# actuday6418/ray-tracer-s8

Hardware: NVIDIA B200
Metric: Mrays/s (higher is better)
Workload: dtype f32

## Files before the change

ray-tracer-s8_b200/csrc/rt_kernels.cu:

```cuda
#include "rt_trace.cuh"
#include "rt_host.h"

#include <algorithm>
#include <cstdio>
#include <cstdlib>
#include <cstring>

namespace rtb {

constexpr int SMEM_TPB = 1024;
constexpr int OUT_SLOTS = 4;
constexpr int TILE_PIX = TILE_W * TILE_H;
constexpr int TILE_BYTES = TILE_PIX * 3;
constexpr uint32_t KEY_FREE = 0xffffffffu;

__device__ __forceinline__ uint32_t smem_u32(const void* p) { return (uint32_t)__cvta_generic_to_shared(p); }
__device__ __forceinline__ void mbar_init(unsigned long long* bar, uint32_t count) {
    asm volatile("mbarrier.init.shared::cta.b64 [%0], %1;" ::"r"(smem_u32(bar)), "r"(count) : "memory");
    asm volatile("fence.mbarrier_init.release.cluster;" ::: "memory");
}
__device__ __forceinline__ void mbar_expect_tx(unsigned long long* bar, uint32_t bytes) {
    asm volatile("mbarrier.arrive.expect_tx.shared::cta.b64 _, [%0], %1;" ::"r"(smem_u32(bar)), "r"(bytes) : "memory");
}
__device__ __forceinline__ void bulk_g2s(void* dst_smem, const void* src_gmem, uint32_t bytes, unsigned long long* bar) {
// ... 20 lines not shown
    unsigned long long* done;
    uint32_t width, out_row0, row0, slab_tile_rows;
};
__device__ __forceinline__ uint32_t slab_of_row(const OutDesc& od, uint32_t y) { return ((y - od.row0) / TILE_H) / od.slab_tile_rows; }

__device__ __forceinline__ void release_count(unsigned long long* done, uint32_t slab, uint32_t cnt) {
    asm volatile("red.release.sys.global.add.u64 [%0], %1;" ::"l"(done + slab), "l"((unsigned long long)cnt) : "memory");
}
__device__ __forceinline__ void count_pixels(const OutDesc& od, uint32_t slab, uint32_t cnt, uint32_t* cntw) {
    if (!od.done || cnt == 0) return;
    if (cntw && (*reinterpret_cast<volatile uint32_t*>(cntw) >> 24) == slab) atomicAdd(cntw, cnt);
    else release_count(od.done, slab, cnt);
}

__device__ __noinline__ void complete_tile(const OutDesc od, const uint8_t* st, uint32_t x0, uint32_t y0, uint32_t valid,
                                           uint32_t hold, uint32_t* cntw) {
    const bool vec = valid == 0xffffffffu && ((od.width & 7u) == 0) && ((reinterpret_cast<uintptr_t>(od.out) & 7u) == 0);
    if (vec) {
#pragma unroll 1
        for (uint32_t r = 0; r < (uint32_t)TILE_H; r++) {
            uint2* dst = reinterpret_cast<uint2*>(od.out + ((size_t)(y0 + r - od.out_row0) * od.width + x0) * 3);
            const uint2* src = reinterpret_cast<const uint2*>(st + r * 24);
            const uint2 v0 = src[0], v1 = src[1], v2 = src[2];
            dst[0] = v0; dst[1] = v1; dst[2] = v2;
        }
    } else {
        for (uint32_t m = valid; m; m &= m - 1u) {
            const uint32_t j = (uint32_t)__ffs(m) - 1u;
            uint8_t* dst = od.out + ((size_t)(y0 + (j >> 3) - od.out_row0) * od.width + x0 + (j & 7u)) * 3;
            dst[0] = st[j * 3 + 0]; dst[1] = st[j * 3 + 1]; dst[2] = st[j * 3 + 2];
        }
    }
    count_pixels(od, slab_of_row(od, y0), (uint32_t)__popc(valid) - hold, cntw);
}

__device__ __noinline__ void evict_tile(const OutDesc od, const uint8_t* st, uint32_t x0, uint32_t y0, uint32_t mask, uint32_t hold,
                                        uint32_t* cntw) {
    const int lane = threadIdx.x & 31;
    if ((mask >> lane) & 1u) {
        const size_t off = ((size_t)(y0 + (lane >> 3) - od.out_row0) * od.width + x0 + (lane & 7)) * 3;
        od.out[off + 0] = st[lane * 3 + 0];
        od.out[off + 1] = st[lane * 3 + 1];
        od.out[off + 2] = st[lane * 3 + 2];
    }
    __syncwarp();
    if (lane == 0) count_pixels(od, slab_of_row(od, y0), (uint32_t)__popc(mask) - hold, cntw);
}

__device__ __noinline__ void store_pixel(const OutDesc od, uint32_t x, uint32_t y, uint32_t rgb, bool count, uint32_t* cntw) {
    const size_t off = ((size_t)(y - od.out_row0) * od.width + x) * 3;
    od.out[off + 0] = (uint8_t)rgb;
    od.out[off + 1] = (uint8_t)(rgb >> 8);
    od.out[off + 2] = (uint8_t)(rgb >> 16);
    if (count) count_pixels(od, slab_of_row(od, y), 1u, cntw);
}

constexpr uint32_t L_HAVE = 1u;           constexpr uint32_t W_TILES_LEFT = 1u;
constexpr uint32_t L_FINISHED = 2u;       constexpr uint32_t W_IN_TAIL = 2u;
                                          constexpr int W_SLOT_SHIFT = 4;
constexpr uint32_t L_REDO = 8u;           constexpr int W_NEXT_SHIFT = 8;
constexpr int L_SLOT_SHIFT = 4;
constexpr uint32_t L_SECOND = 128u;

template <int ISECT, bool SMEM, bool COUNT, bool STAGE, int MINB, int TPB, bool RESUME = false>
__global__ void __launch_bounds__(TPB, MINB) render_kernel_lanes(const DevScene sc, const DevCamera cam,
                                                                const DevParams pr) {
    extern __shared__ float4 smem_dyn[];
    constexpr int NW = TPB / 32;
    __shared__ __align__(16) uint8_t s_stage[STAGE ? NW : 1][OUT_SLOTS][TILE_BYTES];
    __shared__ uint32_t s_key[STAGE ? NW : 1][OUT_SLOTS], s_fill[STAGE ? NW : 1][OUT_SLOTS],
        s_valid[STAGE ? NW : 1][OUT_SLOTS], s_hold[STAGE ? NW : 1][OUT_SLOTS],
        s_cnt[STAGE ? NW : 1];
    __shared__ __align__(8) unsigned long long s_bar;

    const unsigned FULL = 0xffffffffu;
    const int lane = threadIdx.x & 31;
    const int warp = threadIdx.x >> 5;

    SceneView sv;
    if (SMEM) {
        const uint32_t geom = sc.ns * 16u + sc.nt * 64u;
        const uint32_t rest = (ISECT == RT_INTERSECT_BVH) ? sc.lni * (uint32_t)NODE_BYTES
                                                          : ((sc.ns + 7u) & ~7u) * 16u;
        uint8_t* base = reinterpret_cast<uint8_t*>(smem_dyn);
        if (threadIdx.x == 0) mbar_init(&s_bar, 1);
        __syncthreads();
        if (threadIdx.x == 0) {
            mbar_expect_tx(&s_bar, geom + rest);
            if (ISECT == RT_INTERSECT_BVH) {
                bulk_g2s(base, sc.sph, geom + rest, &s_bar);
            } else {
                if (geom) bulk_g2s(base, sc.sph, geom, &s_bar);
                if (rest) bulk_g2s(base + geom, sc.sph2, rest, &s_bar);
            }
        }
        sv.sph = reinterpret_cast<const float4*>(base);
        sv.tri = reinterpret_cast<const float4*>(base + sc.ns * 16u);
        sv.sph2 = reinterpret_cast<const float4*>(base + geom);
        sv.nodes_s = (uint32_t)__cvta_generic_to_shared(base + geom);
        sv.nodes_g = nullptr;
    } else {
        sv.sph2 = sc.sph2;
        sv.sph = sc.sph; sv.tri = sc.tri;
        sv.nodes_s = 0;
        sv.nodes_g = reinterpret_cast<const char*>(sc.lnode);
    }
    if (STAGE && lane < OUT_SLOTS) {
        s_key[warp][lane] = KEY_FREE;
        s_fill[warp][lane] = 0u;
        s_hold[warp][lane] = 0u;
        if (lane == 0) s_cnt[warp] = 0xffu << 24;
    }
    if (SMEM) mbar_wait(&s_bar, 0);
    if (SMEM && ISECT == RT_INTERSECT_BVH) {
        for (uint32_t i = threadIdx.x; i < sc.lni; i += TPB) {
            int2* ch = reinterpret_cast<int2*>(reinterpret_cast<uint8_t*>(smem_dyn) + sc.ns * 16u + sc.nt * 64u +
                                               i * (uint32_t)NODE_BYTES + 48u);
            int2 v = *ch;
            if (v.x >= 0) v.x += (int)sv.nodes_s;
            if (v.y >= 0) v.y += (int)sv.nodes_s;
            *ch = v;
        }
        __syncthreads();
    }
    __syncwarp();

    const unsigned lt_mask = (1u << lane) - 1u;
    const uint32_t total_tiles = pr.tiles_x * pr.tiles_y;
    const uint32_t tail_pixels = pr.pixel_list ? pr.list_count : (pr.my_tickets - pr.tail_first) * (uint32_t)TILE_PIX;
    const float spp_f = (float)pr.spp;

    Ctr ctr;
#pragma unroll
    for (int i = 0; i < NUM_COUNTERS; i++) ctr.v[i] = 0;
    unsigned long long rays = 0;

    uint32_t st = 0;
    uint32_t ws = W_TILES_LEFT | ((uint32_t)TILE_PIX << W_NEXT_SHIFT);
    uint32_t tile_g = 0;
    uint32_t px = 0, py = 0, s = 0, left = 0, np = 0;
    float sr = 0.0f, sg = 0.0f, sb = 0.0f;
    Rng rng;
    rng.s0 = rng.s1 = rng.s2 = rng.s3 = 0;
    V3 o = mk(0, 0, 0), d = mk(0, 0, 1);
    uint32_t path[MAX_PATH];

    auto tile_of_ticket = [&](uint32_t k) -> uint32_t {
        uint32_t g = k * pr.tile_ranks + (pr.tile_rank + k) % pr.tile_ranks;
        if (g < total_tiles) g = total_tiles - 1 - g;
        return g;
    };
    auto out_desc = [&]() { return OutDesc{pr.out, pr.done, pr.width, pr.out_row0, pr.row0, pr.slab_tile_rows}; };

    for (;;) {
        unsigned want = __ballot_sync(FULL, (st & (L_HAVE | L_FINISHED)) == 0);
        if (want) {
            while (want) {
                if (((ws >> W_NEXT_SHIFT) & 63u) >= (uint32_t)TILE_PIX && !(ws & W_IN_TAIL)) {
                    if (!(ws & W_TILES_LEFT)) {
                        if (!(st & L_HAVE)) st |= L_FINISHED;
                        break;
                    }
                    uint32_t k = 0;
                    if (lane == 0) k = atomicAdd(&pr.tile_counter[0], 1u);
                    k = __shfl_sync(FULL, k, 0);
                    const uint32_t g = k < pr.tail_first ? tile_of_ticket(k) : total_tiles;
                    if (g >= total_tiles) {
                        ws |= W_IN_TAIL;
                    } else {
                        tile_g = g;
                        ws &= ~((63u << W_NEXT_SHIFT) | (7u << W_SLOT_SHIFT));
                        if (STAGE) {
                            int sl = -1;
#pragma unroll
                            for (int i = OUT_SLOTS - 1; i >= 0; i--)
                                if (s_key[warp][i] == KEY_FREE) sl = i;
                            if (sl < 0) {
                                sl = (int)(k % OUT_SLOTS);
                                const uint32_t f = s_fill[warp][sl], og = s_key[warp][sl];
                                __syncwarp();
                                if (f) evict_tile(out_desc(), s_stage[warp][sl], (og % pr.tiles_x) * TILE_W,
                                                  pr.row0 + (og / pr.tiles_x) * TILE_H, f, s_hold[warp][sl], &s_cnt[warp]);
                            }
                            const uint32_t x0 = (g % pr.tiles_x) * TILE_W, y0 = pr.row0 + (g / pr.tiles_x) * TILE_H;
                            const uint32_t vm = __ballot_sync(FULL, (x0 + (lane & 7) < pr.width) && (y0 + (lane >> 3) < pr.row1));
                            __syncwarp();
                            if (lane == 0) {
                                s_key[warp][sl] = g;
                                s_fill[warp][sl] = 0u;
                                s_hold[warp][sl] = 0u;
                                s_valid[warp][sl] = vm;
                                const uint32_t slab = ((g / pr.tiles_x) / pr.slab_tile_rows) & 0xffu, w = s_cnt[warp];
                                if ((w >> 24) != slab) {
                                    if (pr.done && (w & 0xffffffu)) release_count(pr.done, w >> 24, w & 0xffffffu);
                                    s_cnt[warp] = slab << 24;
                                }
                            }
                            __syncwarp();
                            ws |= (uint32_t)(sl + 1) << W_SLOT_SHIFT;
                        }
                    }
                }
                uint32_t x = pr.width, y = 0, slot1 = 0, second = 0;
                const uint32_t my = __popc(want & lt_mask);
                const bool wants = (st & (L_HAVE | L_FINISHED)) == 0;
                bool redo_round = false, exhausted = false;
                uint32_t base = 0;
                if (ws & W_IN_TAIL) {
                    if (lane == 0) base = atomicAdd(&pr.tile_counter[1], (unsigned int)__popc(want));
                    base = __shfl_sync(FULL, base, 0);
                    redo_round = exhausted = base >= tail_pixels;
                }
                if (redo_round) {
                    uint32_t t0 = 0, n_take = 0;
                    if (!pr.pixel_list && lane == 0) {
                        int landed = sc.aux_ready;
                        if (!landed) asm volatile("ld.acquire.sys.global.s32 %0, [%1];" : "=r"(landed) : "l"(sc.aux_flag) : "memory");
                        const unsigned long long cnt = *reinterpret_cast<volatile unsigned long long*>(pr.redo_count);
                        if (landed && cnt <= pr.redo_cap) {
                            for (;;) {
                                t0 = *reinterpret_cast<volatile unsigned int*>(&pr.tile_counter[2]);
                                n_take = min((uint32_t)__popc(want), (uint32_t)cnt - min((uint32_t)cnt, t0));
                                if (n_take == 0 || atomicCAS(&pr.tile_counter[2], t0, t0 + n_take) == t0) break;
                            }
                        }
                    }
                    t0 = __shfl_sync(FULL, t0, 0);
                    n_take = __shfl_sync(FULL, n_take, 0);
                    if (n_take == 0 && exhausted) {
                        ws &= ~(W_TILES_LEFT | W_IN_TAIL);
                        if (!(st & L_HAVE)) st |= L_FINISHED;
                        break;
                    }
                    if (n_take) {
                        if (wants && my < n_take) {
                            uint32_t e;
                            for (uint32_t spin = 0;; spin++) {
                                e = *reinterpret_cast<volatile unsigned int*>(&pr.redo_list[t0 + my]);
                                if (e & REDO_VALID) break;
                                if (spin > (1u << 24)) __trap();
                            }
                            e &= ~REDO_VALID;
                            x = e % pr.width;
                            y = e / pr.width;
                            second = L_SECOND;
                        }
                        base = tail_pixels;
                    }
                }
                if (redo_round && base >= tail_pixels) {
                } else if (ws & W_IN_TAIL) {
                    const uint32_t idx = base + my;
                    if (wants && idx < tail_pixels) {
                        if (pr.pixel_list) {
                            const uint32_t p = pr.pixel_list[idx] & ~REDO_VALID;
                            x = p % pr.width;
                            y = p / pr.width;
                        } else {
                            const uint32_t g = tile_of_ticket(pr.tail_first + idx / TILE_PIX);
                            const uint32_t j = idx % TILE_PIX;
                            if (g < total_tiles) {
                                x = (g % pr.tiles_x) * TILE_W + (j & (TILE_W - 1));
                                y = pr.row0 + (g / pr.tiles_x) * TILE_H + (j / TILE_W);
                            }
                        }
                    }
                } else {
                    const uint32_t next = (ws >> W_NEXT_SHIFT) & 63u, avail = (uint32_t)TILE_PIX - next;
                    if (wants && my < avail) {
                        const uint32_t j = next + my;
                        x = (tile_g % pr.tiles_x) * TILE_W + (j & (TILE_W - 1));
                        y = pr.row0 + (tile_g / pr.tiles_x) * TILE_H + (j / TILE_W);
                        slot1 = (ws >> W_SLOT_SHIFT) & 7u;
                    }
                    ws += min((uint32_t)__popc(want), avail) << W_NEXT_SHIFT;
                }
                if (x < pr.width && y < pr.row1) {
                    px = x; py = y;
                    st = L_HAVE | (slot1 << L_SLOT_SHIFT) | second;
                    if constexpr (RESUME) {
                        if (pr.s0 == 0) {
                            rng.seed_from_u64(pr.seed + ((uint64_t)y * pr.width + x));
                            sr = sg = sb = 0.0f;
                        } else {
                            const uint4* rec = pr.state_in + ((size_t)(y - pr.row0) * pr.width + x) * 3;
                            const uint4 a = __ldcs(rec), b = __ldcs(rec + 1), c = __ldcs(rec + 2);
                            rng.s0 = ((uint64_t)a.y << 32) | a.x;
                            rng.s1 = ((uint64_t)a.w << 32) | a.z;
                            rng.s2 = ((uint64_t)b.y << 32) | b.x;
                            rng.s3 = ((uint64_t)b.w << 32) | b.z;
                            sr = __uint_as_float(c.x); sg = __uint_as_float(c.y); sb = __uint_as_float(c.z);
                        }
                        s = pr.s0;
                    } else {
                        rng.seed_from_u64(pr.seed + ((uint64_t)y * pr.width + x));
                        sr = sg = sb = 0.0f;
                        s = 0;
                    }
                    left = 0;
                }
                want = __ballot_sync(FULL, (st & (L_HAVE | L_FINISHED)) == 0);
            }
        }
        if (__ballot_sync(FULL, st & L_HAVE) == 0) break;

        if (st & L_HAVE) {
            if (left == 0) {
                primary_ray(cam, px, pr.height - py - 1, rng, &o, &d);
                left = pr.depth;
                np = 0;
            }
            rays++;
            if (COUNT) {
                ctr.v[CTR_ACTIVE_LANES]++;
                unsigned am = __activemask();
                if (lane == (__ffs(am) - 1)) ctr.v[CTR_TOTAL_LANES] += 32;
            }
            Hit h;
            if (ISECT == RT_INTERSECT_BRUTE) trace_brute<COUNT>(sc, sv, o, d, h, ctr);
            else trace_bvh_ch<COUNT, SMEM>(sc, sv, o, d, h, ctr);
            if (h.unsure) st |= L_REDO;

            bool done;
            float Lr, Lg, Lb;
            if (h.pid >= 0) {
                const float e = __ldg(&sc.emis[h.pid]);
                const float4 m = __ldg(&sc.mat[h.pid]);
                if (e > 0.0f) {
                    Lr = x_mul(m.x, e); Lg = x_mul(m.y, e); Lb = x_mul(m.z, e);
                    done = true;
                    if (COUNT) ctr.v[CTR_EMISSIVE]++;
                } else {
                    V3 n;
                    if (COUNT) ctr.v[h.pid < (int)sc.ns ? CTR_SHADE_SPH : CTR_SHADE_TRI]++;
                    if (h.pid < (int)sc.ns) {
                        n = x_normalize_or_zero(x_sub(h.p, ld3(sv.sph[h.pid])));
                    } else {
                        n = ld3(sv.tri[4 * (h.pid - (int)sc.ns) + 3]);
                    }
                    V3 diffuse = x_add(unit_sphere(rng), n);
                    float kk = x_mul(2.0f, x_dot(d, n));
                    V3 glossy = x_sub(d, x_scale(n, kk));
                    V3 scat = x_add(diffuse, x_scale(x_sub(glossy, diffuse), m.w));
                    const V3 nd = x_normalize_or(scat, n);
                    o = h.p;
                    d = x_normalize_div(nd);
                    path[np++] = (uint32_t)h.pid;
                    left--;
                    done = (left == 0);
                    Lr = Lg = Lb = 0.0f;
                }
            } else {
                if (COUNT) ctr.v[CTR_SKY]++;
                const float ny = x_normalize_or_zero(d).y;
                float t = x_add(x_mul(ny, 0.5f), 1.0f);
                float k1 = x_sub(1.0f, t);
                float w = x_mul(1.0f, t);
                Lr = x_add(w, x_mul(0.3f, k1));
                Lg = Lr;
                Lb = x_add(w, x_mul(0.8f, k1));
                done = true;
            }
            if (done) {
#pragma unroll 1
                while (np > 0) {
                    const float4 m = __ldg(&sc.mat[path[--np]]);
                    Lr = x_mul(m.x, Lr); Lg = x_mul(m.y, Lg); Lb = x_mul(m.z, Lb);
                }
                sr = x_add(sr, Lr); sg = x_add(sg, Lg); sb = x_add(sb, Lb);
                s++;
                left = 0;
                if (s == pr.spp) {
                    if constexpr (RESUME) {
                        if (!(st & L_REDO)) {
                            uint4* rec = pr.state_out + ((size_t)(py - pr.row0) * pr.width + px) * 3;
                            __stcs(rec, make_uint4((uint32_t)rng.s0, (uint32_t)(rng.s0 >> 32), (uint32_t)rng.s1, (uint32_t)(rng.s1 >> 32)));
                            __stcs(rec + 1, make_uint4((uint32_t)rng.s2, (uint32_t)(rng.s2 >> 32), (uint32_t)rng.s3, (uint32_t)(rng.s3 >> 32)));
                            __stcs(rec + 2, make_uint4(__float_as_uint(sr), __float_as_uint(sg), __float_as_uint(sb), 0u));
                        }
                    }
                    const uint32_t rgb = quantise(sr, spp_f) | (quantise(sg, spp_f) << 8) | (quantise(sb, spp_f) << 16);
                    const bool hold = (st & L_REDO) != 0;
                    const int my_sl = (int)((st >> L_SLOT_SHIFT) & 7u) - 1;
                    bool staged = false;
                    if (STAGE && my_sl >= 0) {
                        const uint32_t key = ((py - pr.row0) / TILE_H) * pr.tiles_x + px / TILE_W;
                        if (s_key[warp][my_sl] == key) {
                            const uint32_t j = (px & (TILE_W - 1)) + TILE_W * ((py - pr.row0) & (TILE_H - 1));
                            uint8_t* dst = s_stage[warp][my_sl] + 3 * j;
                            dst[0] = (uint8_t)rgb; dst[1] = (uint8_t)(rgb >> 8); dst[2] = (uint8_t)(rgb >> 16);
                            if (hold) atomicAdd(&s_hold[warp][my_sl], 1u);
                            asm volatile("" ::: "memory");
                            const uint32_t now = atomicOr(&s_fill[warp][my_sl], 1u << j) | (1u << j);
                            if (now == s_valid[warp][my_sl]) {
                                complete_tile(out_desc(), s_stage[warp][my_sl], px & ~(uint32_t)(TILE_W - 1),
                                              py - ((py - pr.row0) & (TILE_H - 1)), now, s_hold[warp][my_sl], &s_cnt[warp]);
                                s_fill[warp][my_sl] = 0u;
                                s_hold[warp][my_sl] = 0u;
                                asm volatile("" ::: "memory");
                                s_key[warp][my_sl] = KEY_FREE;
                            }
                            staged = true;
                        }
                    }
                    if (!staged) store_pixel(out_desc(), px, py, rgb, !hold, STAGE ? &s_cnt[warp] : nullptr);
                    if (st & L_REDO) {
                        atomicAdd(&pr.redo_slab[((py - pr.row0) / TILE_H) / pr.slab_tile_rows], 1ull);
                        const unsigned long long at = atomicAdd(pr.redo_count, 1ull);
                        if (at < pr.redo_cap) pr.redo_list[at] = REDO_VALID | (py * pr.width + px);
                    } else if (st & L_SECOND) {
                        atomicAdd(&pr.redo_slab[((py - pr.row0) / TILE_H) / pr.slab_tile_rows], ~0ull);
                    }
                    st &= ~(L_HAVE | L_REDO | L_SECOND);
                }
            }
        }
    }

    if (STAGE && pr.done) {
        __syncwarp();
        const uint32_t w = s_cnt[warp];
        if (lane == 0 && (w & 0xffffffu)) release_count(pr.done, w >> 24, w & 0xffffffu);
    }
    ctr.v[CTR_RAYS] = rays;
#pragma unroll
    for (int i = 0; i < NUM_COUNTERS; i++) {
        if (!COUNT && i != CTR_RAYS) continue;
        unsigned long long v = ctr.v[i];
#pragma unroll
        for (int ofs = 16; ofs > 0; ofs >>= 1) v += __shfl_down_sync(FULL, v, ofs);
        if (lane == 0 && v) atomicAdd(&pr.counters[i], v);
    }
}

__global__ void wait_slab_kernel(const unsigned long long* done, unsigned long long target, unsigned int* timeout_flag,
                                 unsigned long long max_ns) {
    if (*reinterpret_cast<volatile unsigned int*>(timeout_flag)) return;
    unsigned long long t0;
    asm volatile("mov.u64 %0, %%globaltimer;" : "=l"(t0));
    for (;;) {
        unsigned long long v;
        asm volatile("ld.acquire.sys.global.u64 %0, [%1];" : "=l"(v) : "l"(done) : "memory");
        if (v >= target) return;
        unsigned long long t;
        asm volatile("mov.u64 %0, %%globaltimer;" : "=l"(t));
        if (t - t0 > max_ns) {
            *reinterpret_cast<volatile unsigned int*>(timeout_flag) = 1u;
            __threadfence_system();
            return;
        }
        __nanosleep(200);
    }
}

__global__ void wait_all_slabs_kernel(const unsigned long long* done, unsigned long long seq, uint32_t slabs, uint32_t tile_rows,
                                      uint32_t rows, uint32_t width, unsigned int* timeout_flag, unsigned long long max_ns) {
    const uint32_t s = threadIdx.x;
    if (s >= slabs) return;
    const uint32_t r0 = min(rows, s * tile_rows * (uint32_t)TILE_H), r1 = min(rows, (s + 1) * tile_rows * (uint32_t)TILE_H);
    const unsigned long long target = seq * (unsigned long long)(r1 - r0) * width;
    unsigned long long t0;
    asm volatile("mov.u64 %0, %%globaltimer;" : "=l"(t0));
    for (;;) {
        unsigned long long v;
        asm volatile("ld.acquire.sys.global.u64 %0, [%1];" : "=l"(v) : "l"(done + s) : "memory");
        if (v >= target) return;
        unsigned long long t;
        asm volatile("mov.u64 %0, %%globaltimer;" : "=l"(t));
        if (t - t0 > max_ns) {
            *reinterpret_cast<volatile unsigned int*>(timeout_flag) = 1u;
            __threadfence_system();
            return;
        }
        __nanosleep(200);
    }
}

__global__ void set_u64_kernel(unsigned long long* p, unsigned long long v) {
    __threadfence_system();
    *reinterpret_cast<volatile unsigned long long*>(p) = v;
    __threadfence_system();
}

__global__ void add_counts_kernel(unsigned long long* done, const unsigned long long* add, int n) {
    const int i = threadIdx.x;
    if (i < n && add[i]) {
        __threadfence_system();
        atomicAdd(&done[i], add[i]);
    }
}

__global__ void accum_linear_kernel(const uint4* state, float* out, unsigned long long pixels, float samples) {
    for (unsigned long long i = blockIdx.x * (unsigned long long)blockDim.x + threadIdx.x; i < pixels;
         i += (unsigned long long)gridDim.x * blockDim.x) {
        const uint4 c = state[3 * i + 2];
        out[3 * i + 0] = x_div(__uint_as_float(c.x), samples);
        out[3 * i + 1] = x_div(__uint_as_float(c.y), samples);
        out[3 * i + 2] = x_div(__uint_as_float(c.z), samples);
    }
}

__global__ void __launch_bounds__(256) fp32_peak_kernel(float* out, int iters, float seed) {
    float a0 = seed + threadIdx.x, a1 = a0 + 1, a2 = a0 + 2, a3 = a0 + 3, a4 = a0 + 4, a5 = a0 + 5, a6 = a0 + 6,
          a7 = a0 + 7;
    const float m = 0.999f + seed * 1e-6f, c = 1e-3f + seed;
#pragma unroll 1
    for (int i = 0; i < iters; i++) {
#pragma unroll
        for (int k = 0; k < 16; k++) {
            a0 = fmaf(a0, m, c); a1 = fmaf(a1, m, c); a2 = fmaf(a2, m, c); a3 = fmaf(a3, m, c);
            a4 = fmaf(a4, m, c); a5 = fmaf(a5, m, c); a6 = fmaf(a6, m, c); a7 = fmaf(a7, m, c);
        }
    }
    float r = ((a0 + a1) + (a2 + a3)) + ((a4 + a5) + (a6 + a7));
    if (r == 123.456f) out[blockIdx.x * blockDim.x + threadIdx.x] = r;
}

static int env_int(const char* name, int dflt) {
    const char* e = std::getenv(name);
    return e ? std::atoi(e) : dflt;
}
static bool env_is(const char* name, const char* value) {
    const char* e = std::getenv(name);
    return e && std::strcmp(e, value) == 0;
}
const TestHooks& test_hooks() {
    static const TestHooks t = [] {
        TestHooks v;
        v.build_mode = env_is("RT_B200_BUILD", "host") ? 0 : (env_is("RT_B200_BUILD", "device") ? 2 : 1);
        v.aux_delay_ms = std::max(0, env_int("RT_B200_AUX_DELAY_MS", 0));
        v.wait_timeout_ms = std::max(1, env_int("RT_B200_WAIT_TIMEOUT_MS", 20000));
        v.no_stream_wait = std::getenv("RT_B200_NO_STREAM_WAIT") != nullptr;
        return v;
    }();
    return t;
}

typedef void (*KernelFn)(const DevScene, const DevCamera, const DevParams);

template <int ISECT, bool SMEM>
static KernelFn pick_lanes(bool count, bool stage, int* threads) {
    if (count) {
        *threads = THREADS;
        return (KernelFn)render_kernel_lanes<ISECT, SMEM, true, false, 3, THREADS>;
    }
    if (SMEM) {
        *threads = SMEM_TPB;
        return stage ? (KernelFn)render_kernel_lanes<ISECT, SMEM, false, true, 1, SMEM_TPB>
                     : (KernelFn)render_kernel_lanes<ISECT, SMEM, false, false, 1, SMEM_TPB>;
    }
    *threads = THREADS;
    if (ISECT == RT_INTERSECT_BVH)
        return stage ? (KernelFn)render_kernel_lanes<ISECT, SMEM, false, true, 4, THREADS>
                     : (KernelFn)render_kernel_lanes<ISECT, SMEM, false, false, 4, THREADS>;
    return stage ? (KernelFn)render_kernel_lanes<ISECT, SMEM, false, true, 3, THREADS>
                 : (KernelFn)render_kernel_lanes<ISECT, SMEM, false, false, 3, THREADS>;
}

template <int ISECT, bool SMEM>
static KernelFn pick_resume(int* threads) {
    if constexpr (SMEM) {
        *threads = SMEM_TPB;
        return (KernelFn)render_kernel_lanes<ISECT, SMEM, false, false, 1, SMEM_TPB, true>;
    } else {
        *threads = THREADS;
        if constexpr (ISECT == RT_INTERSECT_BVH) return (KernelFn)render_kernel_lanes<ISECT, SMEM, false, false, 4, THREADS, true>;
        else return (KernelFn)render_kernel_lanes<ISECT, SMEM, false, false, 3, THREADS, true>;
    }
}

size_t scene_smem_bytes(const DevScene& sc, int isect) {
    size_t b = (size_t)sc.ns * 16 + (size_t)sc.nt * 64;
    if (isect == RT_INTERSECT_BVH) b += (size_t)sc.lni * NODE_BYTES;
    else b += (size_t)((sc.ns + 7u) & ~7u) * 16;
    return b;
}

cudaError_t preload_kernels() {
    cudaFuncAttributes a;
    cudaError_t e;
    int th;
#define RT_TOUCH(fn)                                                    \
    if ((e = cudaFuncGetAttributes(&a, fn)) != cudaSuccess) return e;
    for (int count = 0; count < 2; count++)
        for (int stage = 0; stage < 2; stage++) {
            RT_TOUCH((pick_lanes<RT_INTERSECT_BVH, true>(count, stage, &th)));
            RT_TOUCH((pick_lanes<RT_INTERSECT_BVH, false>(count, stage, &th)));
            RT_TOUCH((pick_lanes<RT_INTERSECT_BRUTE, true>(count, stage, &th)));
            RT_TOUCH((pick_lanes<RT_INTERSECT_BRUTE, false>(count, stage, &th)));
        }
    RT_TOUCH((pick_resume<RT_INTERSECT_BVH, true>(&th)));
    RT_TOUCH((pick_resume<RT_INTERSECT_BVH, false>(&th)));
    RT_TOUCH((pick_resume<RT_INTERSECT_BRUTE, true>(&th)));
    RT_TOUCH((pick_resume<RT_INTERSECT_BRUTE, false>(&th)));
    RT_TOUCH(accum_linear_kernel);
    RT_TOUCH(wait_slab_kernel);
    RT_TOUCH(wait_all_slabs_kernel);
    RT_TOUCH(add_counts_kernel);
    RT_TOUCH(set_u64_kernel);
    RT_TOUCH(fp32_peak_kernel);
#undef RT_TOUCH
    return cudaSuccess;
}

constexpr uint64_t kTailPermille = 30;

cudaError_t launch_render(const DevScene& sc, const DevCamera& cam, const DevParams& pr, int isect, bool count,
                          int sm_count, int smem_optin, cudaStream_t stream, LaunchInfo* info) {
    const bool resume = pr.state_out != nullptr;
    if (resume) count = false;
    const size_t static_smem = (SMEM_TPB / 32) * (OUT_SLOTS * (TILE_BYTES + 16) + 4) + 64;
    const size_t need = scene_smem_bytes(sc, isect);
    if (info) info->counts_done = true;
    const bool smem = !count ? (need + static_smem + 1024 <= (size_t)smem_optin)
                             : ((need + static_smem + 1024) * 3 <= (size_t)smem_optin);
    const bool stage = !count && !resume && (pr.tile_ranks > 1 || pr.stage_hint) && pr.done != nullptr;
    int threads = THREADS;
    KernelFn fn;
    if (resume) fn = isect == RT_INTERSECT_BRUTE ? (smem ? pick_resume<RT_INTERSECT_BRUTE, true>(&threads) : pick_resume<RT_INTERSECT_BRUTE, false>(&threads))
                                                 : (smem ? pick_resume<RT_INTERSECT_BVH, true>(&threads) : pick_resume<RT_INTERSECT_BVH, false>(&threads));
    else if (isect == RT_INTERSECT_BRUTE) fn = smem ? pick_lanes<RT_INTERSECT_BRUTE, true>(count, stage, &threads) : pick_lanes<RT_INTERSECT_BRUTE, false>(count, stage, &threads);
    else fn = smem ? pick_lanes<RT_INTERSECT_BVH, true>(count, stage, &threads) : pick_lanes<RT_INTERSECT_BVH, false>(count, stage, &threads);
    const size_t dyn = smem ? need : 0;
// ... 75 lines not shown
```

ray-tracer-s8_b200/csrc/rt_trace.cuh:

```cuda
#pragma once
#include "rt_device.cuh"

namespace rtb {

constexpr int THREADS = 256;

struct Hit {
    float dist;
    int pid;
    V3 p;
    bool unsure;
};
constexpr int HIT_UNSURE = 0x40000000;
__device__ __forceinline__ void hit_finish(Hit& h) {
    h.unsure = h.pid >= 0 && (h.pid & HIT_UNSURE);
    if (h.pid >= 0) h.pid &= ~HIT_UNSURE;
}

struct Ctr {
    unsigned long long v[NUM_COUNTERS];
};

struct SceneView {
    const float4* sph2;
    const float4* sph;
    const float4* tri;
    uint32_t nodes_s;
    const char* nodes_g;
};

#define RT_LDS_F4(v, addr, off) \
    asm volatile("ld.shared.v4.f32 {%0,%1,%2,%3}, [%4+" #off "];" : "=f"((v).x), "=f"((v).y), "=f"((v).z), "=f"((v).w) : "r"(addr))
#define RT_LDS_I2(v, addr, off) asm volatile("ld.shared.v2.s32 {%0,%1}, [%2+" #off "];" : "=r"((v).x), "=r"((v).y) : "r"(addr))

__device__ __forceinline__ bool robustly_inside(V3 p, float t, V3 lo, V3 hi, float extra = 0.0f) {
    const float m0 = fmaf(4e-5f, fabsf(t), extra);
    bool ok = true;
    {
        const float m = fmaf(1e-6f, fabsf(p.x) + fabsf(lo.x) + fabsf(hi.x), m0);
        ok = ok && ((lo.x == hi.x) || ((p.x - lo.x >= m) && (hi.x - p.x >= m)));
    }
    {
        const float m = fmaf(1e-6f, fabsf(p.y) + fabsf(lo.y) + fabsf(hi.y), m0);
        ok = ok && ((lo.y == hi.y) || ((p.y - lo.y >= m) && (hi.y - p.y >= m)));
    }
    {
        const float m = fmaf(1e-6f, fabsf(p.z) + fabsf(lo.z) + fabsf(hi.z), m0);
        ok = ok && ((lo.z == hi.z) || ((p.z - lo.z >= m) && (hi.z - p.z >= m)));
    }
    return ok;
}

struct HitCtx {
    const float4* leaf_box;
    const uint32_t* rank;
    const uint32_t* ref_up;
    const float4* ref_box;
    const int* aux_flag;
    uint32_t n;
    int aux_ready;
};
__device__ __forceinline__ bool aux_now(const HitCtx& hc) {
    if (hc.aux_ready) return true;
    int v;
    asm volatile("ld.acquire.sys.global.s32 %0, [%1];" : "=r"(v) : "l"(hc.aux_flag) : "memory");
    return v != 0;
}
__device__ __forceinline__ HitCtx hit_ctx(const DevScene& sc) {
    return HitCtx{sc.leaf_box, sc.rank, sc.ref_up, sc.ref_box, sc.aux_flag, sc.ns + sc.nt, sc.aux_ready};
}

__device__ __noinline__ bool ref_ancestors_pass(const uint32_t* ref_up, const float4* ref_box, uint32_t n, V3 o, V3 d, int pid) {
    uint32_t u = ref_up[pid];
    while (u != UP_ROOT) {
        u = ref_up[n + (u >> 1)];
        if (u == UP_ROOT) break;
        const V3 lo = ld3(ref_box[2 * u]), hi = ld3(ref_box[2 * u + 1]);
        if (!ref_intersects_aabb(o, d, lo, hi)) return false;
    }
    return true;
}

__device__ __forceinline__ void consider(const HitCtx& hc, V3 o, V3 d, float t, int pid, Hit& best) {
    V3 p = x_add(o, x_scale(d, t));
    int flag = 0;
    if (hc.n > 1) {
        const V3 blo = ld3(__ldg(&hc.leaf_box[2 * pid])), bhi = ld3(__ldg(&hc.leaf_box[2 * pid + 1]));
        const bool degenerate = (d.x == 0.0f) || (d.y == 0.0f) || (d.z == 0.0f);
        if (degenerate) {
            if (!ref_intersects_aabb(o, d, blo, bhi)) return;
            if (!aux_now(hc)) flag = HIT_UNSURE;
            else if (!ref_ancestors_pass(hc.ref_up, hc.ref_box, hc.n, o, d, pid)) return;
        } else if (!robustly_inside(p, t, blo, bhi) && !ref_intersects_aabb(o, d, blo, bhi)) {
            return;
        }
    }
    const V3 po = x_sub(p, o);
    const float dist2 = x_dot(po, po);
    const float dist = x_sqrt_domain(dist2) ? x_sqrt_fast(dist2) : x_sqrt_ool(dist2);
    bool take;
    if (best.pid < 0) {
        take = true;
    } else if (best.dist > dist) {
        take = true;
        flag |= best.pid & HIT_UNSURE;
    } else if (best.dist == dist) {
        if (aux_now(hc)) {
            take = hc.rank[pid] < hc.rank[best.pid & ~HIT_UNSURE];
        } else {
            take = false;
            flag = HIT_UNSURE;
        }
    } else {
        take = false;
    }
    if (take) {
        best.dist = dist;
        best.pid = pid | flag;
        best.p = p;
    } else if (flag) {
        best.pid |= flag;
    }
}

__device__ __forceinline__ bool triangle_filter(const float4* tri, int tidx, V3 o, V3 d, float cull) {
    const V3 a = ld3(tri[4 * tidx + 0]), ab = ld3(tri[4 * tidx + 1]), ac = ld3(tri[4 * tidx + 2]);
    const float ux = fmaf(d.y, ac.z, -ac.y * d.z), uy = fmaf(d.z, ac.x, -ac.z * d.x), uz = fmaf(d.x, ac.y, -ac.x * d.y);
    const float det = fmaf(ab.z, uz, fmaf(ab.y, uy, ab.x * ux));
    const float sdet = fabsf(ab.x * ux) + fabsf(ab.y * uy) + fabsf(ab.z * uz);
    if (fabsf(det) < 1e-5f + 1e-4f * sdet) return true;
    const float inv = __frcp_rn(det), ainv = fabsf(inv);
    const float aox = o.x - a.x, aoy = o.y - a.y, aoz = o.z - a.z;
    const float mag = fabsf(aox) + fabsf(aoy) + fabsf(aoz);
    const float mab = fabsf(ab.x) + fabsf(ab.y) + fabsf(ab.z), mac = fabsf(ac.x) + fabsf(ac.y) + fabsf(ac.z);
    const float u = fmaf(aoz, uz, fmaf(aoy, uy, aox * ux)) * inv;
    const float eu = (1e-4f * (fabsf(aox * ux) + fabsf(aoy * uy) + fabsf(aoz * uz)) + 2e-6f * mag * mac) * ainv + 1e-5f;
    if (u < -eu || u > 1.0f + eu) return false;
    const float vx = fmaf(aoy, ab.z, -ab.y * aoz), vy = fmaf(aoz, ab.x, -ab.z * aox), vz = fmaf(aox, ab.y, -ab.x * aoy);
    const float v = fmaf(d.z, vz, fmaf(d.y, vy, d.x * vx)) * inv;
    const float ev = 1e-4f * mag * mab * ainv + 1e-5f;
    if (v < -ev || u + v > 1.0f + eu + ev) return false;
    const float t = fmaf(ac.z, vz, fmaf(ac.y, vy, ac.x * vx)) * inv;
    const float et = 1e-4f * mag * mab * mac * ainv + 1e-6f;
    if (t < 0.0009f - et || t > cull + et) return false;
    return true;
}

template <bool COUNT>
__device__ __noinline__ void brute_sphere_slow(const HitCtx sc, const float4 s, int pid, V3 o, V3 d, Hit& best,
                                               Ctr& ctr) {
    const V3 oc = mk(x_sub(o.x, s.x), x_sub(o.y, s.y), x_sub(o.z, s.z));
    const float bh = fmaf(oc.z, d.z, fmaf(oc.y, d.y, oc.x * d.x));
    const float oc2 = fmaf(oc.z, oc.z, fmaf(oc.y, oc.y, oc.x * oc.x));
    if (bh > 0.0f && (oc2 - s.w) > 1e-4f * oc2) return;
    if (COUNT) ctr.v[CTR_SPH_EXACT]++;
    float t;
    if (!sphere_root_exact(d, oc, s.w, &t)) return;
    if (COUNT) ctr.v[CTR_SPH_HIT]++;
    consider(sc, o, d, t, pid, best);
}

__device__ __forceinline__ float brute_margin(const float4 s, V3 o, V3 d) {
    const float ocx = x_sub(o.x, s.x), ocy = x_sub(o.y, s.y), ocz = x_sub(o.z, s.z);
    const float bh = fmaf(ocz, d.z, fmaf(ocy, d.y, ocx * d.x));
    const float oc2 = fmaf(ocz, ocz, fmaf(ocy, ocy, ocx * ocx));
    return fmaf(bh, bh, fmaf(oc2, -0.99998f, s.w));
}

template <bool COUNT>
__device__ __noinline__ void brute_group_slow(const HitCtx sc, const float4* sph, const float4* sph2, int first, int count,
                                              V3 o, V3 d, bool all, Hit& best, Ctr& ctr) {
    const f32x2 ox2 = pk2(o.x, o.x), oy2 = pk2(o.y, o.y), oz2 = pk2(o.z, o.z);
    const f32x2 dx2 = pk2(d.x, d.x), dy2 = pk2(d.y, d.y), dz2 = pk2(d.z, d.z);
    const f32x2 kk2 = pk2(-0.99998f, -0.99998f);
    unsigned mask = 0;
#pragma unroll
    for (int k = 0; k < 4; k++) {
        const float4 A = sph2[2 * ((first >> 1) + k)], B = sph2[2 * ((first >> 1) + k) + 1];
        const f32x2 ocx = add2(ox2, pk2(A.x, A.y)), ocy = add2(oy2, pk2(A.z, A.w)), ocz = add2(oz2, pk2(B.x, B.y));
        const f32x2 bh = fma2(ocz, dz2, fma2(ocy, dy2, mul2(ocx, dx2)));
        const f32x2 oc2 = fma2(ocz, ocz, fma2(ocy, ocy, mul2(ocx, ocx)));
        float m_lo, m_hi;
        upk2(fma2(bh, bh, fma2(oc2, kk2, pk2(B.z, B.w))), m_lo, m_hi);
        mask |= (!(m_lo < 0.0f) ? 1u : 0u) << (2 * k);
        mask |= (!(m_hi < 0.0f) ? 1u : 0u) << (2 * k + 1);
    }
    if (all) mask = 0xffu;
    mask &= (1u << count) - 1u;
    while (mask) {
        const int k = __ffs(mask) - 1;
        mask &= mask - 1u;
        brute_sphere_slow<COUNT>(sc, sph[first + k], first + k, o, d, best, ctr);
    }
}

template <bool COUNT>
__device__ __noinline__ void brute_triangle_slow(const HitCtx hc, const float4* tri, int tidx, int pid, V3 o, V3 d, Hit& best, Ctr& ctr) {
    const V3 a = ld3(tri[4 * tidx + 0]), ab = ld3(tri[4 * tidx + 1]), ac = ld3(tri[4 * tidx + 2]);
    if (COUNT) ctr.v[CTR_TRI_TEST]++;
    float t;
    int stage;
    const bool hit = triangle_root_exact(o, d, a, ab, ac, &t, &stage);
    if (COUNT) {
        if (stage >= 1) ctr.v[CTR_TRI_S1]++;
        if (stage >= 2) ctr.v[CTR_TRI_S2]++;
        if (stage >= 3) ctr.v[CTR_TRI_S3]++;
        if (hit) ctr.v[CTR_TRI_HIT]++;
    }
    if (hit) consider(hc, o, d, t, pid, best);
}

template <bool COUNT>
__device__ __forceinline__ void trace_brute_impl(const DevScene& sc, const SceneView& sv, V3 o, V3 d, Hit& best, Ctr& ctr) {
    best.pid = -1;
    best.dist = 0.0f;
    const int ns = (int)sc.ns;
    const bool weird = !(isfinite(o.x) && isfinite(o.y) && isfinite(o.z) && isfinite(d.x) && isfinite(d.y) && isfinite(d.z));
    const f32x2 ox2 = pk2(o.x, o.x), oy2 = pk2(o.y, o.y), oz2 = pk2(o.z, o.z);
    const f32x2 dx2 = pk2(d.x, d.x), dy2 = pk2(d.y, d.y), dz2 = pk2(d.z, d.z);
    const f32x2 kk2 = pk2(-0.99998f, -0.99998f);
    auto pair_margin = [&](int j, float m) {
        const float4 A = sv.sph2[2 * j], B = sv.sph2[2 * j + 1];
        const f32x2 ocx = add2(ox2, pk2(A.x, A.y)), ocy = add2(oy2, pk2(A.z, A.w)), ocz = add2(oz2, pk2(B.x, B.y));
        const f32x2 bh = fma2(ocz, dz2, fma2(ocy, dy2, mul2(ocx, dx2)));
        const f32x2 oc2 = fma2(ocz, ocz, fma2(ocy, ocy, mul2(ocx, ocx)));
        const f32x2 mm = fma2(bh, bh, fma2(oc2, kk2, pk2(B.z, B.w)));
        float m_lo, m_hi;
        upk2(mm, m_lo, m_hi);
        return fmaxf(fmaxf(m, m_lo), m_hi);
    };
    const int ns8 = (ns + 7) & ~7;
    const float NEG = -3.0e38f;
    const HitCtx hc = hit_ctx(sc);
    int i = 0;
    for (; i + 16 <= ns8; i += 16) {
        float m0 = NEG, m1 = NEG;
#pragma unroll
        for (int k = 0; k < 4; k++) {
            m0 = pair_margin((i >> 1) + k, m0);
            m1 = pair_margin((i >> 1) + 4 + k, m1);
        }
        if (COUNT) ctr.v[CTR_SPH_TEST] += min(16, ns - i);
        if (!(fmaxf(m0, m1) < 0.0f) || weird) {
            if (!(m0 < 0.0f) || weird) brute_group_slow<COUNT>(hc, sv.sph, sv.sph2, i, min(8, ns - i), o, d, weird, best, ctr);
            if ((!(m1 < 0.0f) || weird) && i + 8 < ns) brute_group_slow<COUNT>(hc, sv.sph, sv.sph2, i + 8, min(8, ns - i - 8), o, d, weird, best, ctr);
        }
    }
    if (i < ns8) {
        float m0 = NEG;
#pragma unroll
        for (int k = 0; k < 4; k++) m0 = pair_margin((i >> 1) + k, m0);
        if (COUNT) ctr.v[CTR_SPH_TEST] += ns - i;
        if (!(m0 < 0.0f) || weird) brute_group_slow<COUNT>(hc, sv.sph, sv.sph2, i, ns - i, o, d, weird, best, ctr);
    }
    const int nt = (int)sc.nt;
#pragma unroll 1
    for (int j = 0; j < nt; j++) brute_triangle_slow<COUNT>(hc, sv.tri, j, ns + j, o, d, best, ctr);
}

static __device__ __noinline__ float2 camera_uv_slow(float nu, float nv, float u_den, float v_den) {
    return make_float2(x_div_ool(nu, u_den), x_div_ool(nv, v_den));
}
__device__ __forceinline__ void primary_ray(const DevCamera& cam, uint32_t x, uint32_t y_cam, Rng& rng, V3* o_out,
                                            V3* d_out) {
    float a, b;
    unit_disc(rng, a, b);
    V3 offset = mk(x_mul(a, cam.lens_radius), x_mul(b, cam.lens_radius), 0.0f);
    const float nu = x_add((float)x, rng.gen_range_0_1());
    const float nv = x_add((float)y_cam, rng.gen_range_0_1());
    float u = x_quot(nu, cam.u_den, x_rcp_refined(cam.u_den));
    float v = x_quot(nv, cam.v_den, x_rcp_refined(cam.v_den));
    if (!(x_div_num(nu) && x_div_num(nv) && x_div_mag(cam.u_den) && x_div_mag(cam.v_den))) {
        const float2 uv = camera_uv_slow(nu, nv, cam.u_den, cam.v_den);
        u = uv.x;
        v = uv.y;
    }
    V3 org = mk(cam.org[0], cam.org[1], cam.org[2]);
    V3 llc = mk(cam.llc[0], cam.llc[1], cam.llc[2]);
    V3 hor = mk(cam.hor[0], cam.hor[1], cam.hor[2]);
    V3 ver = mk(cam.ver[0], cam.ver[1], cam.ver[2]);
    V3 target = x_sub(x_add(x_add(llc, x_scale(hor, u)), x_scale(ver, v)), org);
    V3 d1 = x_normalize_div_or_zero(target);
    V3 focal_point = x_add(org, x_scale(d1, cam.focus));
    V3 fo = x_add(org, offset);
    *o_out = fo;
    *d_out = x_normalize_div_or_zero(x_sub(focal_point, fo));
}

static __device__ __noinline__ float x_sqrt_div_slow(float a, float b) { return x_sqrt_ool(x_div_ool(a, b)); }
__device__ __forceinline__ uint32_t quantise(float sum, float spp_f) {
    const float m = x_quot(sum, spp_f, x_rcp_refined(spp_f));
    float c = (m == 0.0f) ? m : x_sqrt_fast(m);
    if (!(x_div_num(sum) && x_div_mag(spp_f) && (m == 0.0f || x_sqrt_domain(m)))) c = x_sqrt_div_slow(sum, spp_f);
    float s = x_mul(c, 255.999f);
    uint32_t q = __float2uint_rz(s);
    return q > 255u ? 255u : q;
}

template <bool SMEM>
__device__ __forceinline__ void load_node(const SceneView& sv, int cur, float4& a, float4& b, float4& c, int2& ch) {
    if (SMEM) {
        RT_LDS_F4(a, cur, 0);
        RT_LDS_F4(b, cur, 16);
        RT_LDS_F4(c, cur, 32);
        RT_LDS_I2(ch, cur, 48);
    } else {
        const float4* nrec = reinterpret_cast<const float4*>(sv.nodes_g + cur);
        a = __ldg(nrec); b = __ldg(nrec + 1); c = __ldg(nrec + 2);
        ch = __ldg(reinterpret_cast<const int2*>(nrec + 3));
    }
}
constexpr int TR_DONE = (int)0x80000000;
template <bool COUNT, bool SMEM>
__device__ __forceinline__ void trace_bvh_ch_impl(const DevScene& sc, const SceneView& sv, V3 o, V3 d, Hit& best, Ctr& ctr) {
    best.pid = -1;
    best.dist = 0.0f;
    const float BIG = 1e30f;
    float ix = fminf(fmaxf(__frcp_rn(d.x), -BIG), BIG);
    float iy = fminf(fmaxf(__frcp_rn(d.y), -BIG), BIG);
    float iz = fminf(fmaxf(__frcp_rn(d.z), -BIG), BIG);
    if (!(fabsf(d.x) > 0.0f)) ix = BIG;
    if (!(fabsf(d.y) > 0.0f)) iy = BIG;
    if (!(fabsf(d.z) > 0.0f)) iz = BIG;
    const float ax = fabsf(ix), ay = fabsf(iy), az = fabsf(iz);
    const float qx = -o.x * ix, qy = -o.y * iy, qz = -o.z * iz;
    const float slack = 4.8e-7f * fmaxf(fmaxf(fabsf(qx), fabsf(qy)), fabsf(qz)) + 1e-30f;
    const f32x2 i_xy = pk2(ix, iy), q_xy = pk2(qx, qy), a_xy = pk2(ax, ay), na_xy = pk2(-ax, -ay);
    const f32x2 i_zz = pk2(iz, iz), q_zz = pk2(qz, qz), a_zz = pk2(az, az), na_zz = pk2(-az, -az);
    const f32x2 slack2 = pk2(slack, slack);
    float cull = 1001.0f;
    const int ns = (int)sc.ns;
    const HitCtx hc = hit_ctx(sc);
    int stack[MAX_STACK + 1 + MAX_BIG];
    stack[0] = TR_DONE;
    int* top = stack + 1;
    if (sc.ltree) *top++ = (SMEM && sc.lroot >= 0) ? sc.lroot + (int)sv.nodes_s : sc.lroot;
#pragma unroll 1
    for (int i = (int)sc.nbig - 1; i >= 0; i--) *top++ = __ldg(&sc.big_code[i]);
    int cur = *--top;
    for (;;) {
        while (cur >= 0) {
            float4 a, b, c;
            int2 ch;
            load_node<SMEM>(sv, cur, a, b, c, ch);
            const f32x2 lc2 = fma2(pk2(a.x, a.y), i_xy, q_xy), rc2 = fma2(pk2(b.x, b.y), i_xy, q_xy);
            const f32x2 ln2 = fma2(na_xy, pk2(a.z, a.w), lc2), lf2 = fma2(a_xy, pk2(a.z, a.w), lc2);
            const f32x2 rn2 = fma2(na_xy, pk2(b.z, b.w), rc2), rf2 = fma2(a_xy, pk2(b.z, b.w), rc2);
            const f32x2 cz2 = fma2(pk2(c.x, c.y), i_zz, q_zz);
            const f32x2 nz2 = fma2(na_zz, pk2(c.z, c.w), cz2), fz2 = fma2(a_zz, pk2(c.z, c.w), cz2);
            float lnx, lny, lfx, lfy, rnx, rny, rfx, rfy, lnz, rnz, lfz, rfz;
            upk2(ln2, lnx, lny); upk2(lf2, lfx, lfy); upk2(rn2, rnx, rny); upk2(rf2, rfx, rfy);
            upk2(nz2, lnz, rnz); upk2(fz2, lfz, rfz);
            const float tl = fmaxf(fmaxf(lnx, lny), fmaxf(lnz, 0.0f));
            const float fl = fminf(fminf(lfx, lfy), fminf(lfz, cull));
            const float tr = fmaxf(fmaxf(rnx, rny), fmaxf(rnz, 0.0f));
            const float fr = fminf(fminf(rfx, rfy), fminf(rfz, cull));
            float fls, frs;
            upk2(add2(pk2(fl, fr), slack2), fls, frs);
            const bool hl = tl <= fls;
            const bool hr = tr <= frs;
            if (COUNT) ctr.v[CTR_SLAB] += 2;
            const bool swap = tr < tl;
            if (hl && hr) *top++ = swap ? ch.x : ch.y;
            int nxt = (hr && (!hl || swap)) ? ch.y : ch.x;
            if (!(hl || hr)) nxt = *--top;
            cur = nxt;
        }
        if (cur == TR_DONE) return;
        const int pid = (~cur) >> 5;
        float t = 0.0f;
        bool cand = false;
        if (pid < ns) {
            const float4 s = sv.sph[pid];
            const V3 oc = mk(x_sub(o.x, s.x), x_sub(o.y, s.y), x_sub(o.z, s.z));
            const float bh = fmaf(oc.z, d.z, fmaf(oc.y, d.y, oc.x * d.x));
            const float oc2 = fmaf(oc.z, oc.z, fmaf(oc.y, oc.y, oc.x * oc.x));
            const float cf = oc2 - s.w;
            const float disc = fmaf(bh, bh, -cf);
            if (COUNT) ctr.v[CTR_SPH_TEST]++;
            if (!(fmaf(oc2, 2e-5f, disc) < 0.0f) && !(bh > 0.0f && cf > 1e-4f * oc2)) {
                if (COUNT) ctr.v[CTR_SPH_EXACT]++;
                cand = sphere_root_exact(d, oc, s.w, &t);
                if (COUNT && cand) ctr.v[CTR_SPH_HIT]++;
            }
        } else {
            if (COUNT) ctr.v[CTR_TRI_TEST]++;
            if (triangle_filter(sv.tri, pid - ns, o, d, cull)) {
                const V3 a = ld3(sv.tri[4 * (pid - ns) + 0]), ab = ld3(sv.tri[4 * (pid - ns) + 1]), ac = ld3(sv.tri[4 * (pid - ns) + 2]);
                int stage;
                cand = triangle_root_exact(o, d, a, ab, ac, &t, &stage);
                if (COUNT) {
                    if (stage >= 1) ctr.v[CTR_TRI_S1]++;
                    if (stage >= 2) ctr.v[CTR_TRI_S2]++;
                    if (stage >= 3) ctr.v[CTR_TRI_S3]++;
                    if (cand) ctr.v[CTR_TRI_HIT]++;
                }
            }
        }
        if (cand) {
            consider(hc, o, d, t, pid, best);
            cull = fmaf(best.dist, 1.00001f, 1e-6f);
        }
        cur = *--top;
    }
}

template <bool COUNT>
__device__ __forceinline__ void trace_brute(const DevScene& sc, const SceneView& sv, V3 o, V3 d, Hit& best, Ctr& ctr) {
    trace_brute_impl<COUNT>(sc, sv, o, d, best, ctr);
    hit_finish(best);
}
template <bool COUNT, bool SMEM>
__device__ __forceinline__ void trace_bvh_ch(const DevScene& sc, const SceneView& sv, V3 o, V3 d, Hit& best, Ctr& ctr) {
    trace_bvh_ch_impl<COUNT, SMEM>(sc, sv, o, d, best, ctr);
    hit_finish(best);
}

}
```

Measured before the change: 6896.

## Prefilter big primitives before BVH traversal and pad warp stacks to align

Large out-of-tree primitives are now run through the cheap sphere and triangle filters once, up front, and only the ones that pass are pushed onto the traversal stack. Each lane then pads its stack with no-op entries up to the warp-wide maximum count, so lanes pop the real entries in step. Leaf entries carry a flag bit that decides whether the filter runs again before the exact root test. This aims to cut divergent per-leaf filter work for big primitives, at the cost of an extra warp reduction and wasted padding pops. It also relies on tree leaf codes having the unfiltered bit set correctly; that host-side code is not shown.

Measured after the change: 6870, median of 6. No clear change (-0.4%).

```diff
diff --git a/ray-tracer-s8_b200/csrc/rt_kernels.cu b/ray-tracer-s8_b200/csrc/rt_kernels.cu
--- a/ray-tracer-s8_b200/csrc/rt_kernels.cu
+++ b/ray-tracer-s8_b200/csrc/rt_kernels.cu
@@ -346,7 +346,8 @@
                 want = __ballot_sync(FULL, (st & (L_HAVE | L_FINISHED)) == 0);
             }
         }
-        if (__ballot_sync(FULL, st & L_HAVE) == 0) break;
+        const unsigned busy = __ballot_sync(FULL, st & L_HAVE);
+        if (busy == 0) break;
 
         if (st & L_HAVE) {
             if (left == 0) {
@@ -362,7 +363,7 @@
             }
             Hit h;
             if (ISECT == RT_INTERSECT_BRUTE) trace_brute<COUNT>(sc, sv, o, d, h, ctr);
-            else trace_bvh_ch<COUNT, SMEM>(sc, sv, o, d, h, ctr);
+            else trace_bvh_ch<COUNT, SMEM>(sc, sv, o, d, h, ctr, busy);
             if (h.unsure) st |= L_REDO;
 
             bool done;
diff --git a/ray-tracer-s8_b200/csrc/rt_trace.cuh b/ray-tracer-s8_b200/csrc/rt_trace.cuh
--- a/ray-tracer-s8_b200/csrc/rt_trace.cuh
+++ b/ray-tracer-s8_b200/csrc/rt_trace.cuh
@@ -123,8 +123,15 @@
     }
 }
 
-__device__ __forceinline__ bool triangle_filter(const float4* tri, int tidx, V3 o, V3 d, float cull) {
-    const V3 a = ld3(tri[4 * tidx + 0]), ab = ld3(tri[4 * tidx + 1]), ac = ld3(tri[4 * tidx + 2]);
+__device__ __forceinline__ bool sphere_filter(V3 oc, V3 d, float r2) {
+    const float bh = fmaf(oc.z, d.z, fmaf(oc.y, d.y, oc.x * d.x));
+    const float oc2 = fmaf(oc.z, oc.z, fmaf(oc.y, oc.y, oc.x * oc.x));
+    const float cf = oc2 - r2;
+    const float disc = fmaf(bh, bh, -cf);
+    return !(fmaf(oc2, 2e-5f, disc) < 0.0f) && !(bh > 0.0f && cf > 1e-4f * oc2);
+}
+
+__device__ __forceinline__ bool triangle_filter(V3 a, V3 ab, V3 ac, V3 o, V3 d, float cull) {
     const float ux = fmaf(d.y, ac.z, -ac.y * d.z), uy = fmaf(d.z, ac.x, -ac.z * d.x), uz = fmaf(d.x, ac.y, -ac.x * d.y);
     const float det = fmaf(ab.z, uz, fmaf(ab.y, uy, ab.x * ux));
     const float sdet = fabsf(ab.x * ux) + fabsf(ab.y * uy) + fabsf(ab.z * uz);
@@ -144,6 +151,9 @@
     const float et = 1e-4f * mag * mab * mac * ainv + 1e-6f;
     if (t < 0.0009f - et || t > cull + et) return false;
     return true;
+}
+__device__ __forceinline__ bool triangle_filter(const float4* tri, int tidx, V3 o, V3 d, float cull) {
+    return triangle_filter(ld3(tri[4 * tidx + 0]), ld3(tri[4 * tidx + 1]), ld3(tri[4 * tidx + 2]), o, d, cull);
 }
 
 template <bool COUNT>
@@ -311,10 +321,40 @@
     }
 }
 constexpr int TR_DONE = (int)0x80000000;
+constexpr int LEAF_UNFILTERED = 1;
+constexpr int TR_PAD = ~2;
 template <bool COUNT, bool SMEM>
-__device__ __forceinline__ void trace_bvh_ch_impl(const DevScene& sc, const SceneView& sv, V3 o, V3 d, Hit& best, Ctr& ctr) {
+__device__ __forceinline__ void trace_bvh_ch_impl(const DevScene& sc, const SceneView& sv, V3 o, V3 d, Hit& best, Ctr& ctr,
+                                                  unsigned lanes) {
     best.pid = -1;
     best.dist = 0.0f;
+    float cull = 1001.0f;
+    const int ns = (int)sc.ns;
+    int stack[MAX_STACK + 1 + MAX_BIG];
+    stack[0] = TR_DONE;
+    int* top = stack + 1;
+    if (sc.ltree) *top++ = (SMEM && sc.lroot >= 0) ? sc.lroot + (int)sv.nodes_s : sc.lroot;
+    int nc = 0;
+#pragma unroll 1
+    for (int i = (int)sc.nbig - 1; i >= 0; i--) {
+        const int code = __ldg(&sc.big_code[i]);
+        const int pid = (~code) >> 5;
+        bool pass;
+        if (pid < ns) {
+            const float4 s = sv.sph[pid];
+            if (COUNT) ctr.v[CTR_SPH_TEST]++;
+            pass = sphere_filter(mk(x_sub(o.x, s.x), x_sub(o.y, s.y), x_sub(o.z, s.z)), d, s.w);
+        } else {
+            if (COUNT) ctr.v[CTR_TRI_TEST]++;
+            pass = triangle_filter(sv.tri, pid - ns, o, d, cull);
+        }
+        if (pass) {
+            *top++ = code & ~LEAF_UNFILTERED;
+            nc++;
+        }
+    }
+#pragma unroll 1
+    for (int k = __reduce_max_sync(lanes, nc) - nc; k > 0; k--) *top++ = TR_PAD;
     const float BIG = 1e30f;
     float ix = fminf(fmaxf(__frcp_rn(d.x), -BIG), BIG);
     float iy = fminf(fmaxf(__frcp_rn(d.y), -BIG), BIG);
@@ -328,15 +368,7 @@
     const f32x2 i_xy = pk2(ix, iy), q_xy = pk2(qx, qy), a_xy = pk2(ax, ay), na_xy = pk2(-ax, -ay);
     const f32x2 i_zz = pk2(iz, iz), q_zz = pk2(qz, qz), a_zz = pk2(az, az), na_zz = pk2(-az, -az);
     const f32x2 slack2 = pk2(slack, slack);
-    float cull = 1001.0f;
-    const int ns = (int)sc.ns;
     const HitCtx hc = hit_ctx(sc);
-    int stack[MAX_STACK + 1 + MAX_BIG];
-    stack[0] = TR_DONE;
-    int* top = stack + 1;
-    if (sc.ltree) *top++ = (SMEM && sc.lroot >= 0) ? sc.lroot + (int)sv.nodes_s : sc.lroot;
-#pragma unroll 1
-    for (int i = (int)sc.nbig - 1; i >= 0; i--) *top++ = __ldg(&sc.big_code[i]);
     int cur = *--top;
     for (;;) {
         while (cur >= 0) {
@@ -367,39 +399,38 @@
             cur = nxt;
         }
         if (cur == TR_DONE) return;
-        const int pid = (~cur) >> 5;
-        float t = 0.0f;
-        bool cand = false;
-        if (pid < ns) {
-            const float4 s = sv.sph[pid];
-            const V3 oc = mk(x_sub(o.x, s.x), x_sub(o.y, s.y), x_sub(o.z, s.z));
-            const float bh = fmaf(oc.z, d.z, fmaf(oc.y, d.y, oc.x * d.x));
-            const float oc2 = fmaf(oc.z, oc.z, fmaf(oc.y, oc.y, oc.x * oc.x));
-            const float cf = oc2 - s.w;
-            const float disc = fmaf(bh, bh, -cf);
-            if (COUNT) ctr.v[CTR_SPH_TEST]++;
-            if (!(fmaf(oc2, 2e-5f, disc) < 0.0f) && !(bh > 0.0f && cf > 1e-4f * oc2)) {
-                if (COUNT) ctr.v[CTR_SPH_EXACT]++;
-                cand = sphere_root_exact(d, oc, s.w, &t);
-                if (COUNT && cand) ctr.v[CTR_SPH_HIT]++;
-            }
-        } else {
-            if (COUNT) ctr.v[CTR_TRI_TEST]++;
-            if (triangle_filter(sv.tri, pid - ns, o, d, cull)) {
+        if (cur != TR_PAD) {
+            const int pid = (~cur) >> 5;
+            const bool filtered = !(cur & LEAF_UNFILTERED);
+            float t = 0.0f;
+            bool cand = false;
+            if (pid < ns) {
+                const float4 s = sv.sph[pid];
+                const V3 oc = mk(x_sub(o.x, s.x), x_sub(o.y, s.y), x_sub(o.z, s.z));
+                if (COUNT && !filtered) ctr.v[CTR_SPH_TEST]++;
+                if (sphere_filter(oc, d, s.w) || filtered) {
+                    if (COUNT) ctr.v[CTR_SPH_EXACT]++;
+                    cand = sphere_root_exact(d, oc, s.w, &t);
+                    if (COUNT && cand) ctr.v[CTR_SPH_HIT]++;
+                }
+            } else {
+                if (COUNT && !filtered) ctr.v[CTR_TRI_TEST]++;
                 const V3 a = ld3(sv.tri[4 * (pid - ns) + 0]), ab = ld3(sv.tri[4 * (pid - ns) + 1]), ac = ld3(sv.tri[4 * (pid - ns) + 2]);
-                int stage;
-                cand = triangle_root_exact(o, d, a, ab, ac, &t, &stage);
-                if (COUNT) {
-                    if (stage >= 1) ctr.v[CTR_TRI_S1]++;
-                    if (stage >= 2) ctr.v[CTR_TRI_S2]++;
-                    if (stage >= 3) ctr.v[CTR_TRI_S3]++;
-                    if (cand) ctr.v[CTR_TRI_HIT]++;
+                if (filtered || triangle_filter(a, ab, ac, o, d, cull)) {
+                    int stage;
+                    cand = triangle_root_exact(o, d, a, ab, ac, &t, &stage);
+                    if (COUNT) {
+                        if (stage >= 1) ctr.v[CTR_TRI_S1]++;
+                        if (stage >= 2) ctr.v[CTR_TRI_S2]++;
+                        if (stage >= 3) ctr.v[CTR_TRI_S3]++;
+                        if (cand) ctr.v[CTR_TRI_HIT]++;
+                    }
                 }
             }
-        }
-        if (cand) {
-            consider(hc, o, d, t, pid, best);
-            cull = fmaf(best.dist, 1.00001f, 1e-6f);
+            if (cand) {
+                consider(hc, o, d, t, pid, best);
+                cull = fmaf(best.dist, 1.00001f, 1e-6f);
+            }
         }
         cur = *--top;
     }
@@ -411,8 +442,9 @@
     hit_finish(best);
 }
 template <bool COUNT, bool SMEM>
-__device__ __forceinline__ void trace_bvh_ch(const DevScene& sc, const SceneView& sv, V3 o, V3 d, Hit& best, Ctr& ctr) {
-    trace_bvh_ch_impl<COUNT, SMEM>(sc, sv, o, d, best, ctr);
+__device__ __forceinline__ void trace_bvh_ch(const DevScene& sc, const SceneView& sv, V3 o, V3 d, Hit& best, Ctr& ctr,
+                                             unsigned lanes) {
+    trace_bvh_ch_impl<COUNT, SMEM>(sc, sv, o, d, best, ctr, lanes);
     hit_finish(best);
 }
 
```
